# apache/datafusion-ballista

Hardware: NVIDIA H100
Metric: tpch_q1_rows_per_sec (higher is better)
Workload: dtype decimal128/i128

## Files before the change

datafusion-ballista_b200/csrc/host/engine.cpp:

```cpp
#include <sched.h>
#include <sys/stat.h>

#include <algorithm>
#include <atomic>
#include <cctype>
#include <chrono>
#include <cmath>
#include <cstdio>
#include <map>
#include <mutex>
#include <functional>
#include <set>

#include "../common/arrow_host.hpp"
#include "../common/tpch_gen.hpp"
#include "../device/kernels.h"
#include "host_pool.hpp"
#include "lower.hpp"
#include "nccl_dyn.hpp"
#include "../common/plan_proto.hpp"
#include "../common/plan_dump.hpp"
#include "parquet_meta.hpp"
#include "arrow_ipc.hpp"

// ... 25 lines not shown
  std::string name;
  uint64_t output_rows = 0, input_rows = 0, elapsed_ns = 0, bytes_read = 0, bytes_written = 0, launches = 0;
};

}

struct b200_engine {
  int device = 0;
  int rank = 0, world = 1;
  int sm_count = 132;
  cudaStream_t own_stream = nullptr;
  cudaStream_t stream = nullptr;
  std::mutex mu;
  std::map<std::string, std::map<int, DevBatchPtr>> tables;
  std::map<ShuffleKey, std::vector<Piece>> shuffle;
  std::atomic<uint64_t> launches{0};
  std::atomic<uint64_t> n_fused{0}, n_fused_static{0}, n_vm{0}, n_groupby{0}, n_groupby_pf{0}, n_fastfilter{0};
  int64_t batch_size = 8192;
  std::map<std::string, std::string> config;
  std::map<std::string, int> agg_hint;
  uint64_t pf_bucket_slots = (uint64_t)1 << 19;
  int64_t pf_min_rows = (int64_t)1 << 22;
  std::map<std::string, uint64_t> agg_groups;
  void* pinned_stage = nullptr;
  std::unique_ptr<HostPool> pool;
  std::mutex ingest_mu;
  struct NarrowSlot {
    void* pinned = nullptr;
    void* dev = nullptr;
    cudaEvent_t done = nullptr;
    bool used = false;
    size_t bytes = 0;
  } nslot[4];
  int64_t ingest_chunk_rows = (int64_t)1 << 22;
  int ingest_slots = 3;
  bool kernel_timing = false;
  struct KernelSample { std::string name; cudaEvent_t e0, e1; uint64_t bytes; };
  std::vector<KernelSample> ksamples;
  struct KernelStat { double ms = 0; uint64_t launches = 0, bytes = 0; };
  std::map<std::string, KernelStat> kstats;
  ncclComm_t comm = nullptr;
  std::mutex comm_mu;
  uint64_t exch_sent_bytes = 0, exch_recv_bytes = 0;
  size_t win_config_bytes = 0;
  uint8_t* win_local = nullptr;
  size_t win_bytes = 0, win_used = 0;
  std::vector<uint8_t*> win_peer;
  uint64_t fused_exchanges = 0;
  std::mutex export_mu;
  uint8_t* export_arena = nullptr;
  std::atomic<uint64_t> narrowed_bytes_saved{0};
  std::atomic<uint64_t> n_window_sorts{0};
  std::atomic<uint64_t> nlj_pairs{0};
};

struct b200_stage {
  b200_engine* eng = nullptr;
  std::string job_id;
  int64_t stage_id = 0;
  PlanPtr plan;
  std::string fingerprint;
  std::vector<OpMetrics> metrics;
  std::map<const PlanNode*, int> metric_index;
};

#define NCCL_CHECK(expr)                                                                                              \
  do {                                                                                                                \
    ncclResult_t _r = (expr);                                                                                         \
    if (_r != 0) throw EngineError(B200_ERR_CUDA, std::string("NCCL error: ") + NcclApi::get().GetErrorString(_r) + " at " + __FILE__ + ":" + std::to_string(__LINE__)); \
  } while (0)

static void release_window(b200_engine* e);
static void setup_window(b200_engine* e);

namespace {

struct TaskCtx {
  uint8_t* arena = nullptr;
  size_t pos = 0;
  bool drained = true;
  std::vector<std::function<void()>> checks;
};
static const size_t TASK_ARENA_BYTES = (size_t)1 << 16;
inline TaskCtx& task_ctx() {
  static thread_local TaskCtx t;
  if (!t.arena && cudaHostAlloc((void**)&t.arena, TASK_ARENA_BYTES, cudaHostAllocDefault) != cudaSuccess) t.arena = nullptr;
  return t;
}

struct Exec {
  b200_engine* e;
  b200_stage* s;
  const volatile int32_t* cancel;
  cudaStream_t st() const { return e->stream; }
  void check_cancel() const {
    if (cancel && *cancel) throw EngineError(B200_ERR_CANCELLED, "task cancelled");
  }
  OpMetrics* m(const PlanNode* n) const {
    if (!s) return nullptr;
    auto it = s->metric_index.find(n);
    return it == s->metric_index.end() ? nullptr : &s->metrics[(size_t)it->second];
  }
  const void* fetch_bytes(const void* dptr, size_t bytes) const {
    TaskCtx& t = task_ctx();
    if (!t.arena) throw EngineError(B200_ERR_OOM, "pinned read-back arena unavailable");
    if (t.drained) {
      t.pos = 0;
      t.drained = false;
    }
    const size_t at = (t.pos + 15) & ~(size_t)15;
    if (at + bytes > TASK_ARENA_BYTES) {
      sync();
      return fetch_bytes(dptr, bytes);
    }
    CUDA_CHECK(cudaMemcpyAsync(t.arena + at, dptr, bytes, cudaMemcpyDeviceToHost, st()));
    t.pos = at + bytes;
    return t.arena + at;
  }
  void* stage_bytes(size_t bytes) const {
    TaskCtx& t = task_ctx();
    if (!t.arena) throw EngineError(B200_ERR_OOM, "pinned staging arena unavailable");
    if (t.drained) {
      t.pos = 0;
      t.drained = false;
    }
    size_t at = (t.pos + 15) & ~(size_t)15;
    if (at + bytes > TASK_ARENA_BYTES) {
      sync();
      t.pos = 0;
      t.drained = false;
      at = 0;
      if (bytes > TASK_ARENA_BYTES) throw EngineError(B200_ERR_INVALID, "staging request larger than the arena");
    }
    t.pos = at + bytes;
    return t.arena + at;
  }
  template <class T>
  const T* fetch(const void* dptr) const {
    return (const T*)fetch_bytes(dptr, sizeof(T));
  }
  void defer(std::function<void()> fn) const { task_ctx().checks.push_back(std::move(fn)); }
  void sync() const {
    TaskCtx& t = task_ctx();
    cudaError_t se = cudaStreamSynchronize(st());
    t.drained = true;
    std::vector<std::function<void()>> cs;
    cs.swap(t.checks);
    CUDA_CHECK(se);
    for (auto& c : cs) c();
    check_cancel();
  }
  static void abandon() {
    TaskCtx& t = task_ctx();
    t.checks.clear();
    t.drained = true;
  }
  template <class T>
  T get(const void* dptr) const {
    const T* p = fetch<T>(dptr);
    sync();
    return *p;
  }
};

struct KernelTimer {
  b200_engine* e;
  cudaStream_t st;
  b200_engine::KernelSample ks;
  bool on;
  KernelTimer(const Exec& x, const char* name, uint64_t bytes) : e(x.e), st(x.st()), on(x.e->kernel_timing) {
    if (!on) return;
    ks.name = name;
    ks.bytes = bytes;
    if (cudaEventCreate(&ks.e0) != cudaSuccess || cudaEventCreate(&ks.e1) != cudaSuccess) {
      on = false;
      return;
    }
    cudaEventRecord(ks.e0, st);
  }
  ~KernelTimer() {
    if (!on) return;
    cudaEventRecord(ks.e1, st);
    std::lock_guard<std::mutex> g(e->mu);
    e->ksamples.push_back(ks);
  }
};

struct ScopeTimer {
  const char* name;
  std::chrono::steady_clock::time_point t0;
  bool on;
  explicit ScopeTimer(const char* n) : name(n) {
    static const bool enabled = getenv("B200_TIMING") != nullptr;
    on = enabled;
    if (on) t0 = std::chrono::steady_clock::now();
  }
  ~ScopeTimer() {
// ... 449 lines not shown
    if (hcs[ci].type.id == TypeId::Utf8) {
      int32_t total = 0;
      memcpy(&total, arena + slots[ci].data + (size_t)n * 4, 4);
      if ((size_t)total > slots[ci].chars_cap) return false;
    }
  for (size_t ci = 0; ci < b.cols.size(); ci++) {
    HostCol& h = hcs[ci];
    const Slot& sl = slots[ci];
    if (sl.has_valid) {
      unsigned long long nulls = 0;
      memcpy(&nulls, arena + sl.count, 8);
      h.null_count = (int64_t)nulls;
      if (nulls) h.validity.assign(arena + sl.validity, arena + sl.validity + (size_t)(n + 7) / 8);
    }
    if (!h.data.empty()) memcpy(h.data.data(), arena + sl.data, h.data.size());
    if (h.type.id == TypeId::Utf8) {
      const int32_t total = ((const int32_t*)h.data.data())[n];
      h.extra.assign(arena + sl.chars, arena + sl.chars + (size_t)total);
    }
  }
  hcs_out = std::move(hcs);
  return true;
}

std::vector<HostCol> download_batch(const Exec& x, const DevBatch& b, int64_t r0, int64_t r1) {
  const int64_t n = r1 - r0;
  std::vector<HostCol> hcs;
  if (n <= SMALL_EXPORT_ROWS && download_small(x, b, r0, r1, hcs)) return hcs;
  hcs.clear();
  cudaStream_t st = x.st();
  for (auto& c0 : b.cols) {
    DevColumn c = slice_column(c0, r0, r1);
    HostCol h;
    h.name = c.name;
    h.type = c.type;
    h.nullable = true;
    h.n = n;
    if (c.valid && n) {
      DevPtr bm = dev_alloc((size_t)(n + 7) / 8 + 16, st);
      DevPtr cnt = dev_alloc(8, st);
      CUDA_CHECK(cudaMemsetAsync(cnt->ptr, 0, 8, st));
      launch_bytes_to_bitmap(c.valid, (uint8_t*)bm->ptr, n, (unsigned long long*)cnt->ptr, st);
      h.validity.resize((size_t)(n + 7) / 8);
      CUDA_CHECK(cudaMemcpyAsync(h.validity.data(), bm->ptr, h.validity.size(), cudaMemcpyDeviceToHost, st));
      h.null_count = (int64_t)x.get<unsigned long long>(cnt->ptr);
      if (h.null_count == 0) h.validity.clear();
    }
    if (c.type.id == TypeId::Bool) {
      h.data.assign((size_t)(n + 7) / 8, 0);
      if (n) {
        DevPtr bm = dev_alloc((size_t)(n + 7) / 8 + 16, st);
        launch_bytes_to_bitmap(c.data, (uint8_t*)bm->ptr, n, nullptr, st);
        CUDA_CHECK(cudaMemcpyAsync(h.data.data(), bm->ptr, h.data.size(), cudaMemcpyDeviceToHost, st));
        CUDA_CHECK(cudaStreamSynchronize(st));
      }
    } else if (c.type.id == TypeId::Utf8) {
      DevColumn u = c.phys == PH_STRVIEW ? as_utf8(x, c) : c;
      h.data.resize((size_t)(n + 1) * 4);
      CUDA_CHECK(cudaMemcpyAsync(h.data.data(), u.data, h.data.size(), cudaMemcpyDeviceToHost, st));
      CUDA_CHECK(cudaStreamSynchronize(st));
      int32_t* off = (int32_t*)h.data.data();
      int32_t first = off[0], last = off[n];
      h.extra.resize((size_t)(last - first));
      if (last > first) CUDA_CHECK(cudaMemcpyAsync(h.extra.data(), u.chars + first, h.extra.size(), cudaMemcpyDeviceToHost, st));
      CUDA_CHECK(cudaStreamSynchronize(st));
      for (int64_t i = 0; i <= n; i++) off[i] -= first;
    } else {
      h.data.resize((size_t)n * c.width());
      if (n) CUDA_CHECK(cudaMemcpyAsync(h.data.data(), c.data, h.data.size(), cudaMemcpyDeviceToHost, st));
      CUDA_CHECK(cudaStreamSynchronize(st));
    }
    hcs.push_back(std::move(h));
  }
  return hcs;
}

void export_batch(const Exec& x, const DevBatch& b, int64_t r0, int64_t r1, ArrowArray* out, ArrowSchema* out_schema) {
  std::vector<HostCol> hcs = download_batch(x, b, r0, r1);
  export_record_batch(std::move(hcs), r1 - r0, out, out_schema);
}

struct RunOutcome {
  RunStatus status;
  float ms = 0;
};

struct FusedPlan {
  FusedSpec spec;
  FusedShape shape;
  int block = 0;
  size_t smem = 0;
};

static void throw_run_error(unsigned int error) {
  if (error == 1) throw EngineError(B200_ERR_EXECUTION, "Arithmetic overflow");
  if (error == 2) throw EngineError(B200_ERR_EXECUTION, "Divide by zero");
  if (error) throw EngineError(B200_ERR_EXECUTION, "execution error in expression");
}

static bool program_filters(const Program& P) {
  for (int i = 0; i < P.n_instr; i++)
    if (P.code[i].op == OP_FILTER || (P.code[i].flags & IF_FILTER)) return true;
  return false;
}

bool match_groupby(const Program& P, GroupBySpec& S);
bool match_fast_filter(const Program& P, FastFilterSpec& S);

bool partition_for_groupby(const Exec& x, GroupBySpec& S, std::vector<DevPtr>& keep) {
  const uint64_t GB_PF_BUCKET_SLOTS = x.e->pf_bucket_slots;
  if (!GB_PF_BUCKET_SLOTS || S.n_keys < 1 || S.table.cap < GB_PF_BUCKET_SLOTS * 8 || S.n_rows < x.e->pf_min_rows || S.n_rows >= ((int64_t)1 << 32)) return false;
  for (int k = 0; k < S.n_keys; k++) {
    const uint32_t w = S.cols[S.key_col[k]].width;
    if (w != 4 && w != 8) return false;
  }
  const uint32_t K = (uint32_t)std::min<uint64_t>(S.table.cap / GB_PF_BUCKET_SLOTS, PART_MAX_FANOUT);
  const int64_t n = S.n_rows;
  PidSrc ps;
  memset(&ps, 0, sizeof ps);
  ps.salt = 0x5bd1e995;
  for (int k = 0; k < S.n_keys; k++) {
    const FusedCol& c = S.cols[S.key_col[k]];
    ps.keys[ps.n_keys++] = KeyCol{c.data, nullptr, (uint8_t)(c.width == 4 ? PH_I32 : PH_I64), (uint8_t)c.width};
// ... 1616 lines not shown
      case PlanNode::Passthrough:
        out = (n.op_name == "CoalescePartitionsExec") ? exec_all(*n.children[0]) : exec(*n.children[0], part);
        break;
      case PlanNode::Limit: {
        DevBatchPtr in = (n.op_name == "GlobalLimitExec") ? exec_all(*n.children[0]) : exec(*n.children[0], part);
        int64_t r0 = std::min<int64_t>(std::max<int64_t>(0, n.skip), in->n);
        int64_t r1 = n.fetch >= 0 ? std::min<int64_t>(in->n, r0 + n.fetch) : in->n;
        out = std::make_shared<DevBatch>();
        out->n = r1 - r0;
        for (auto& c : in->cols) out->cols.push_back(slice_column(c, r0, r1));
        break;
      }
      case PlanNode::Window: out = exec_window(n, part, met); break;
      case PlanNode::ShuffleWriter: throw EngineError(B200_ERR_INVALID, "nested ShuffleWriterExec");
    }
    if (met) met->output_rows += (uint64_t)out->n;
    return out;
  }

  DevBatchPtr do_sort(const std::vector<SortKey>& keys, int64_t fetch, DevBatchPtr in, OpMetrics* met) {
    const int64_t n = in->n;
    auto t0 = std::chrono::steady_clock::now();
    std::vector<DevColumn> kcols;
    bool need_eval = false;
    for (auto& k : keys) need_eval |= k.expr->kind != Expr::Col;
    DevBatchPtr work = in;
    size_t n_in_cols = in->cols.size();
    if (need_eval && n > 0) {
      PipelineBuilder pb(*in, x.st());
      std::vector<ColRef> outs = pb.cols;
      for (auto& k : keys) {
        ColRef c = pb.compile(*k.expr);
        pb.pin(c);
        outs.push_back(c);
      }
      work = run_materialize(x, pb, outs, in, met);
      for (size_t k = 0; k < keys.size(); k++) kcols.push_back(work->cols[n_in_cols + k]);
    } else {
      for (auto& k : keys) kcols.push_back(in->cols.at((size_t)(k.expr->kind == Expr::Col ? k.expr->col : 0)));
    }
    if (n <= 1 || keys.empty()) {
      auto out = std::make_shared<DevBatch>();
      int64_t m = fetch >= 0 ? std::min<int64_t>(fetch, n) : n;
      out->n = m;
      for (size_t c = 0; c < n_in_cols; c++) out->cols.push_back(slice_column(in->cols[c], 0, m));
      return out;
    }
    const int64_t m = fetch >= 0 ? std::min<int64_t>(fetch, n) : n;
    DevPtr idx = sort_permutation(keys, kcols, n, m);
    DevBatch proj;
    proj.n = n;
    for (size_t c = 0; c < n_in_cols; c++) proj.cols.push_back(in->cols[c]);
    DevBatchPtr out = gather_batch(x, proj, (const int64_t*)idx->ptr, m, false);
    if (n > SMALL_SORT_MAX_ROWS || keys.size() > (size_t)SMALL_SORT_MAX_KEYS) CUDA_CHECK(cudaStreamSynchronize(x.st()));
    if (met) {
      met->elapsed_ns += (uint64_t)std::chrono::duration_cast<std::chrono::nanoseconds>(std::chrono::steady_clock::now() - t0).count();
      met->input_rows += (uint64_t)n;
    }
    return out;
  }

  static bool window_input_sorted(const PlanNode& n) {
    const PlanNode* c = n.children[0].get();
    while (c->op == PlanNode::Passthrough && c->op_name == "CoalesceBatchesExec") c = c->children[0].get();
    if (c->op != PlanNode::Sort && c->op != PlanNode::SortPreservingMerge) return false;
    const size_t np = n.window_partition.size(), no = n.window_order.size();
    if (c->sort_keys.size() != np + no) return false;
    auto in_sort_prefix = [&](const ExprPtr& e) {
      for (size_t k = 0; k < np; k++)
        if (expr_equal(c->sort_keys[k].expr, e)) return true;
      return false;
    };
    for (size_t k = 0; k < np; k++) {
      bool found = false;
      for (auto& pk : n.window_partition) found = found || expr_equal(c->sort_keys[k].expr, pk);
      if (!found || !in_sort_prefix(n.window_partition[k])) return false;
    }
    for (size_t k = 0; k < no; k++) {
      const SortKey &a = c->sort_keys[np + k], &b = n.window_order[k];
      if (!expr_equal(a.expr, b.expr) || a.asc != b.asc || a.nulls_first != b.nulls_first) return false;
    }
    return true;
  }

  DevBatchPtr exec_window(const PlanNode& n, int part, OpMetrics* met) {
    DevBatchPtr in = exec(*n.children[0], part);
    const auto t0 = std::chrono::steady_clock::now();
    const int64_t N = in->n;
    if (N >= ((int64_t)1 << 32)) throw EngineError(B200_ERR_UNSUPPORTED, "window over " + std::to_string(N) + " rows (the sort takes at most 2^32)");
    const size_t np = n.window_partition.size(), no = n.window_order.size(), nw = n.window_exprs.size();
    if (np + no > (size_t)WIN_MAX_KEYS) throw EngineError(B200_ERR_UNSUPPORTED, "window with more than " + std::to_string(WIN_MAX_KEYS) + " partition and order keys");
    auto out = std::make_shared<DevBatch>();
    out->n = N;
    out->cols = in->cols;
    const size_t n_in = in->cols.size();
    if (met) met->input_rows += (uint64_t)N;
    if (N == 0) {
      for (size_t w = 0; w < nw; w++) {
        const Field& f = n.schema[n_in + w];
        DevColumn c = make_out_column(f.name, f.type, f.type.id == TypeId::Utf8 ? PH_STRVIEW : phys_of(f.type), 0, f.nullable, x.st());
        c.n = 0;
        out->cols.push_back(c);
      }
      return out;
    }
    std::vector<ExprPtr> exprs(n.window_partition);
    for (auto& k : n.window_order) exprs.push_back(k.expr);
// ... 213 lines not shown
      }
      DevPtr fv, fc, bv, bc, tiles;
      {
        KernelTimer kt(x, "window_scan", (uint64_t)N * ((arg ? (uint64_t)arg->width() + 1 : 0) + (perm ? 8 : 0) + vw + 1) +
                                             (uint64_t)N * (fwd + bwd) * 2 * (vw + 1 + 8 + vw + 4));
        launch_window_load(L, perm, N, x.st());
        WinScan S;
        memset(&S, 0, sizeof S);
        S.vals = vals->ptr;
        S.valid = (const uint8_t*)valid->ptr;
        S.n = N;
        S.w = std::max<int64_t>(E.w, 1);
        S.acc = E.acc;
        S.op = E.op;
        S.seg = seg;
        if (fwd || bwd) tiles = dev_alloc((size_t)window_scan_tile_bytes(N), x.st());
        S.tiles = tiles ? tiles->ptr : nullptr;
        if (fwd) {
          fv = dev_alloc((size_t)N * vw, x.st());
          fc = dev_alloc((size_t)N * 4, x.st());
          S.out_v = fv->ptr;
          S.out_c = (uint32_t*)fc->ptr;
          S.dir = 0;
          launch_window_scan(S, B, x.st());
          E.fwd_v = fv->ptr;
          E.fwd_c = (const uint32_t*)fc->ptr;
        }
        x.check_cancel();
        if (bwd) {
          bv = dev_alloc((size_t)N * vw, x.st());
          bc = dev_alloc((size_t)N * 4, x.st());
          S.out_v = bv->ptr;
          S.out_c = (uint32_t*)bc->ptr;
          S.dir = 1;
          launch_window_scan(S, B, x.st());
          E.bwd_v = bv->ptr;
          E.bwd_c = (const uint32_t*)bc->ptr;
        }
      }
      if (E.fin == WFIN_AVG && E.acc == WACC_I128) {
        if (!error) {
          error = dev_alloc(16, x.st());
          CUDA_CHECK(cudaMemsetAsync(error->ptr, 0, 16, x.st()));
        }
        E.error = (unsigned int*)error->ptr;
      }
      {
        KernelTimer kt(x, "window_frames", (uint64_t)N * (32 + 2 * (vw + 4) + (perm ? 8 : 0) + (uint64_t)oc.width() + 1));
        launch_window_eval(E, B, perm, N, x.st());
      }
      out->cols.push_back(oc);
    }
    if (error && x.get<unsigned int>(error->ptr)) throw EngineError(B200_ERR_EXECUTION, "Arithmetic overflow in a window AVG over Decimal128");
    CUDA_CHECK(cudaStreamSynchronize(x.st()));
    if (met) met->elapsed_ns += (uint64_t)std::chrono::duration_cast<std::chrono::nanoseconds>(std::chrono::steady_clock::now() - t0).count();
    return out;
  }

  DevPtr sort_permutation(const std::vector<SortKey>& keys, const std::vector<DevColumn>& kcols, int64_t n, int64_t m) {
    if (n >= ((int64_t)1 << 32)) throw EngineError(B200_ERR_UNSUPPORTED, "sort of more than 2^32 rows");
    if (n <= SMALL_SORT_MAX_ROWS && keys.size() <= (size_t)SMALL_SORT_MAX_KEYS) {
      SmallSortKeys K;
      K.n_keys = (int)keys.size();
      std::vector<DevColumn> kv;
      for (size_t ki = 0; ki < keys.size(); ki++) {
        kv.push_back(as_views(x, kcols[ki]));
        const DevColumn& kc = kv.back();
        SortWordArgs& A = K.k[ki];
        A.data = kc.data;
        A.valid = kc.valid;
        A.phys = kc.phys;
        A.asc = keys[ki].asc;
        A.nulls_first = keys[ki].nulls_first;
        A.word = 0;
      }
      DevPtr idx = dev_alloc((size_t)n * 8, x.st());
      launch_small_sort(K, (int64_t*)idx->ptr, n, x.st());
      return idx;
    }
    const uint32_t n_blocks = (uint32_t)((n + 2047) / 2048);
    DevPtr ka = dev_alloc((size_t)n * 8, x.st()), kb = dev_alloc((size_t)n * 8, x.st());
    DevPtr va = dev_alloc((size_t)n * 4, x.st()), vb = dev_alloc((size_t)n * 4, x.st());
    DevPtr hist = dev_alloc((size_t)256 * n_blocks * 4 + 64, x.st());
    DevPtr scan = dev_alloc(((size_t)256 * n_blocks + 1 + (size_t)(256 * n_blocks) / 1024 + 8) * 8, x.st());
    uint32_t* perm = (uint32_t*)va->ptr;
    launch_iota_u32(perm, n, x.st());
    for (size_t ki = keys.size(); ki-- > 0;) {
      DevColumn kc = as_views(x, kcols[ki]);
      int n_words = 1;
      if (kc.phys == PH_DEC128) n_words = 2;
      if (kc.phys == PH_STRVIEW) {
        DevPtr mx = dev_alloc(16, x.st());
        CUDA_CHECK(cudaMemsetAsync(mx->ptr, 0, 16, x.st()));
        launch_max_view_len((const unsigned long long*)kc.data, kc.valid, n, (unsigned int*)mx->ptr, x.st());
        unsigned int maxlen = x.get<unsigned int>(mx->ptr);
        n_words = (int)(maxlen / 7) + 1;
      }
      for (int w = n_words - 1; w >= (kc.valid ? -1 : 0); w--) {
        x.check_cancel();
        SortWordArgs A;
        A.data = kc.data;
        A.valid = kc.valid;
        A.phys = kc.phys;
        A.asc = keys[ki].asc;
        A.nulls_first = keys[ki].nulls_first;
        A.word = w;
        uint64_t* kin = (uint64_t*)ka->ptr;
// ... 1687 lines not shown
    return B200_OK;
  } catch (const EngineError& e) {
    g_err = e.what();
    return e.code;
  } catch (const PlanUnsupported& e) {
    g_err = e.what();
    return B200_ERR_UNSUPPORTED;
  } catch (const std::bad_alloc&) {
    g_err = "host out of memory";
    return B200_ERR_OOM;
  } catch (const std::exception& e) {
    g_err = e.what();
    return B200_ERR_INVALID;
  } catch (...) {
    g_err = "unknown error";
    return B200_ERR_INVALID;
  }
}

template <class F>
int guard(b200_engine* e, F&& f) {
  const uint64_t l0 = launches_on_thread();
  const int rc = guard(std::forward<F>(f));
  if (e) e->launches += launches_on_thread() - l0;
  return rc;
}

}

static void release_window(b200_engine* e) {
  for (size_t d = 0; d < e->win_peer.size(); d++)
    if (e->win_peer[d] && (int)d != e->rank) cudaIpcCloseMemHandle(e->win_peer[d]);
  e->win_peer.clear();
  if (e->win_local) cudaFree(e->win_local);
  e->win_local = nullptr;
  e->win_bytes = e->win_used = 0;
}

static void comm_allgather(b200_engine* e, const void* mine, void* all, size_t rec) {
  NcclApi& N = NcclApi::get();
  const int W = e->world, me = e->rank;
  uint8_t* dev = nullptr;
  CUDA_CHECK(cudaMalloc((void**)&dev, rec * (size_t)W));
  try {
    CUDA_CHECK(cudaMemcpyAsync(dev + rec * (size_t)me, mine, rec, cudaMemcpyHostToDevice, e->stream));
    NCCL_CHECK(N.GroupStart());
    for (int d = 0; d < W; d++) {
      if (d == me) continue;
      NCCL_CHECK(N.Send(dev + rec * (size_t)me, rec, kNcclUint8, d, e->comm, e->stream));
      NCCL_CHECK(N.Recv(dev + rec * (size_t)d, rec, kNcclUint8, d, e->comm, e->stream));
    }
    NCCL_CHECK(N.GroupEnd());
    CUDA_CHECK(cudaMemcpyAsync(all, dev, rec * (size_t)W, cudaMemcpyDeviceToHost, e->stream));
    CUDA_CHECK(cudaStreamSynchronize(e->stream));
  } catch (...) {
    cudaFree(dev);
    throw;
  }
  cudaFree(dev);
}

static void setup_window(b200_engine* e) {
  const int W = e->world, me = e->rank;
  struct Rec {
    cudaIpcMemHandle_t h;
    uint64_t bytes, ok;
  };
  Rec mine;
  memset(&mine, 0, sizeof mine);
  const size_t want = (e->win_config_bytes + 4095) & ~(size_t)4095;
  uint8_t* ptr = nullptr;
  if (cudaMalloc((void**)&ptr, want) == cudaSuccess && cudaIpcGetMemHandle(&mine.h, ptr) == cudaSuccess) {
    mine.bytes = want;
    mine.ok = 1;
  } else {
    cudaGetLastError();
    if (ptr) cudaFree(ptr);
    ptr = nullptr;
  }
  std::vector<Rec> all((size_t)W);
  comm_allgather(e, &mine, all.data(), sizeof(Rec));
  bool ok = true;
  for (auto& r : all) ok = ok && r.ok && r.bytes == want;
  std::vector<uint8_t*> peer((size_t)W, nullptr);
  if (ok) {
    for (int d = 0; d < W && ok; d++) {
      if (d == me) {
        peer[(size_t)d] = ptr;
        continue;
      }
      void* m = nullptr;
      if (cudaIpcOpenMemHandle(&m, all[(size_t)d].h, cudaIpcMemLazyEnablePeerAccess) != cudaSuccess) {
        cudaGetLastError();
        ok = false;
      }
      peer[(size_t)d] = (uint8_t*)m;
    }
  }
  uint64_t flag = ok ? 1 : 0;
  std::vector<uint64_t> flags((size_t)W, 0);
  comm_allgather(e, &flag, flags.data(), sizeof flag);
  for (uint64_t f : flags) ok = ok && f;
  if (!ok) {
    for (int d = 0; d < W; d++)
      if (d != me && peer[(size_t)d]) cudaIpcCloseMemHandle(peer[(size_t)d]);
    if (ptr) cudaFree(ptr);
    return;
// ... 72 lines not shown
    CUDA_CHECK(cudaDeviceGetDefaultMemPool(&pool, device));
    uint64_t thr = pool_bytes ? pool_bytes : UINT64_MAX;
    CUDA_CHECK(cudaMemPoolSetAttribute(pool, cudaMemPoolAttrReleaseThreshold, &thr));
    *out = e;
  });
}

void b200_engine_destroy(b200_engine* e) {
  if (!e) return;
  cudaSetDevice(e->device);
  cudaStreamSynchronize(e->stream);
  e->tables.clear();
  e->shuffle.clear();
  cudaStreamSynchronize(e->stream);
  for (auto& sl : e->nslot) {
    if (sl.pinned) cudaFreeHost(sl.pinned);
    if (sl.dev) cudaFree(sl.dev);
    if (sl.done) cudaEventDestroy(sl.done);
  }
  release_window(e);
  if (e->comm && NcclApi::get().ok()) NcclApi::get().CommDestroy(e->comm);
  if (e->export_arena) cudaFreeHost(e->export_arena);
  if (arena_chunk() && arena_chunk()->stream == e->own_stream) arena_chunk().reset();
  if (e->own_stream) cudaStreamDestroy(e->own_stream);
  delete e;
}

int b200_engine_set_stream(b200_engine* e, void* cuda_stream) {
  return guard([&] {
    CUDA_CHECK(cudaStreamSynchronize(e->stream));
    e->stream = cuda_stream ? (cudaStream_t)cuda_stream : e->own_stream;
  });
}
int b200_engine_synchronize(b200_engine* e) {
  return guard([&] {
    CUDA_CHECK(cudaSetDevice(e->device));
    CUDA_CHECK(cudaStreamSynchronize(e->stream));
  });
}
uint64_t b200_engine_kernel_launches(b200_engine* e) { return e->launches; }
uint64_t b200_engine_counter(b200_engine* e, const char* name) {
  const std::string n = name ? name : "";
  if (n == "fused") return e->n_fused;
  if (n == "groupby_partition_first") return e->n_groupby_pf;
  if (n == "fused_static") return e->n_fused_static;
  if (n == "fused_exchanges") return e->fused_exchanges;
  if (n == "exchange_window_bytes") return e->win_bytes;
  if (n == "vm") return e->n_vm;
  if (n == "groupby") return e->n_groupby;
  if (n == "fastfilter") return e->n_fastfilter;
  if (n == "ingest_bytes_saved") return e->narrowed_bytes_saved;
  if (n == "nlj_pairs") return e->nlj_pairs;
  if (n == "window_sorts") return e->n_window_sorts;
  return 0;
}

int b200_engine_set_config(b200_engine* e, const char* key, const char* value) {
  return guard([&] {
    std::lock_guard<std::mutex> g(e->mu);
    e->config[key] = value;
    if (std::string(key) == "datafusion.execution.batch_size") e->batch_size = std::max<int64_t>(1, atoll(value));
    if (std::string(key) == "b200.ingest.chunk_rows") e->ingest_chunk_rows = std::max<int64_t>(1 << 16, atoll(value));
    if (std::string(key) == "b200.ingest.slots") e->ingest_slots = atoi(value);
    if (std::string(key) == "b200.exchange.window_bytes") e->win_config_bytes = (size_t)strtoull(value, nullptr, 10);
    if (std::string(key) == "b200.ingest.threads") e->pool.reset();
    if (std::string(key) == "b200.agg.partition_first.bucket_slots") {
      const uint64_t v = strtoull(value, nullptr, 10);
      e->pf_bucket_slots = v ? std::max<uint64_t>(next_pow2(v), 64) : 0;
    }
    if (std::string(key) == "b200.agg.partition_first.min_rows") e->pf_min_rows = std::max<int64_t>(1, atoll(value));
    if (std::string(key) == "b200.agg.reset_hints") {
      e->agg_hint.clear();
      e->agg_groups.clear();
    }
    if (std::string(key) == "b200.metrics.kernel_timing") e->kernel_timing = std::string(value) == "on" || std::string(value) == "1" || std::string(value) == "true";
  });
}

int b200_engine_register_batch(b200_engine* e, const char* table, int partition, struct ArrowArray* batch, struct ArrowSchema* schema) {
  return guard(e, [&] {
    CUDA_CHECK(cudaSetDevice(e->device));
    DevBatchPtr b = import_batch(e, batch, schema);
    Exec x{e, nullptr, nullptr};
    build_column_images(x, *b);
    DevBatchPtr prev;
    {
      std::lock_guard<std::mutex> g(e->mu);
      auto& slot = e->tables[table][partition];
      prev = slot;
      if (!prev) slot = b;
    }
    if (prev) {
      Runner r{x, ""};
      Schema s;
      for (auto& c : prev->cols) s.push_back(Field{c.name, c.type, true});
      DevBatchPtr cat = r.concat({prev, b}, s);
      for (auto& c : cat->cols) c = as_utf8(x, c);
      build_column_images(x, *cat);
      CUDA_CHECK(cudaStreamSynchronize(e->stream));
      std::lock_guard<std::mutex> g(e->mu);
      e->tables[table][partition] = cat;
    }
  });
}

int b200_engine_drop_table(b200_engine* e, const char* table) {
// ... 154 lines not shown
int b200_engine_register_parquet(b200_engine* e, const char* table, int partition, const char* path, const char* columns_csv) {
  return guard(e, [&] {
    if (!e || !table || !path) throw EngineError(B200_ERR_INVALID, "null argument");
    CUDA_CHECK(cudaSetDevice(e->device));
    std::vector<std::string> cols;
    if (columns_csv && *columns_csv) {
      std::string sct(columns_csv);
      size_t p = 0;
      while (p <= sct.size()) {
        size_t q = sct.find(',', p);
        if (q == std::string::npos) q = sct.size();
        if (q > p) cols.push_back(sct.substr(p, q - p));
        p = q + 1;
      }
    }
    Exec x{e, nullptr, nullptr};
    DevBatchPtr b;
    try {
      b = scan_parquet(x, path, cols);
    } catch (...) {
      cudaStreamSynchronize(e->stream);
      Exec::abandon();
      throw;
    }
    std::lock_guard<std::mutex> g(e->mu);
    e->tables[table][partition] = b;
  });
}

int64_t b200_tpch_table_rows(const char* table, int64_t msf) {
  const int t = table ? table_id(table) : -1;
  return t < 0 ? -1 : tpch::table_rows(t, msf);
}

int b200_engine_export_table(b200_engine* e, const char* table, int partition, struct ArrowArray* out, struct ArrowSchema* out_schema) {
  return guard(e, [&] {
    CUDA_CHECK(cudaSetDevice(e->device));
    DevBatchPtr b;
    {
      std::lock_guard<std::mutex> g(e->mu);
      auto it = e->tables.find(table);
      if (it == e->tables.end() || !it->second.count(partition)) throw EngineError(B200_ERR_NOT_FOUND, "no such table partition");
      b = it->second[partition];
    }
    Exec x{e, nullptr, nullptr};
    export_batch(x, *b, 0, b->n, out, out_schema);
  });
}

int b200_stage_prepare(b200_engine* e, const char* job_id, int64_t stage_id, const char* plan_json, uint64_t plan_len, b200_stage** out) {
  ScopeTimer tm("stage_prepare");
  return guard([&] {
    if (!e || !plan_json || !out) throw EngineError(B200_ERR_INVALID, "null argument");
    Json j = parse_json(plan_json, plan_len ? (size_t)plan_len : strlen(plan_json));
    PlanPtr plan = parse_plan(j);
    if (plan->op != PlanNode::ShuffleWriter)
      throw EngineError(B200_ERR_INVALID, "Plan passed to new_query_stage_exec is not a ShuffleWriterExec");
    auto* s = new b200_stage();
    s->eng = e;
    s->job_id = job_id ? job_id : plan->job_id;
    s->stage_id = stage_id;
    plan->stage_id = stage_id;
    {
      std::string shape(plan_json, plan_len ? (size_t)plan_len : strlen(plan_json));
      const std::string tag = "\"job_id\":\"";
      size_t at = shape.find(tag);
      if (at != std::string::npos) {
        size_t end = shape.find('"', at + tag.size());
        if (end != std::string::npos) shape.erase(at + tag.size(), end - at - tag.size());
      }
      s->fingerprint = std::to_string(stage_id) + ":" + std::to_string(mix64(hash_bytes((const uint8_t*)shape.data(), (uint32_t)shape.size())));
    }
    collect_nodes(*plan, s);
    s->plan = std::move(plan);
    *out = s;
  });
}

int b200_plan_proto_to_json(const void* plan_bytes, uint64_t n_bytes, const char* job_id, char** out_json) {
  return guard([&] {
    if (!plan_bytes || !out_json) throw EngineError(B200_ERR_INVALID, "null argument");
    std::string js;
    try {
      js = pbp::plan_proto_to_json(plan_bytes, (size_t)n_bytes, job_id ? std::string(job_id) : std::string());
    } catch (const pbp::Unsupported& u) {
      throw EngineError(B200_ERR_UNSUPPORTED, u.what());
    } catch (const std::runtime_error& r) {
      throw EngineError(B200_ERR_INVALID, r.what());
    }
    char* m = (char*)malloc(js.size() + 1);
    if (!m) throw EngineError(B200_ERR_OOM, "plan JSON");
    memcpy(m, js.c_str(), js.size() + 1);
    *out_json = m;
  });
}

void b200_string_free(char* s) { free(s); }

int b200_plan_typed_json(const char* plan_json, uint64_t plan_len, char** out_json) {
  return guard([&] {
    if (!plan_json || !out_json) throw EngineError(B200_ERR_INVALID, "null argument");
    Json j = parse_json(plan_json, plan_len ? (size_t)plan_len : strlen(plan_json));
    PlanPtr plan = parse_plan(j);
    const std::string js = dump_plan(*plan);
    char* m = (char*)malloc(js.size() + 1);
    if (!m) throw EngineError(B200_ERR_OOM, "plan JSON");
    memcpy(m, js.c_str(), js.size() + 1);
    *out_json = m;
  });
}

int b200_stage_prepare_proto(b200_engine* e, const char* job_id, int64_t stage_id, const void* plan_bytes, uint64_t n_bytes, b200_stage** out) {
  char* js = nullptr;
  int rc = b200_plan_proto_to_json(plan_bytes, n_bytes, job_id, &js);
  if (rc != 0) return rc;
  rc = b200_stage_prepare(e, job_id, stage_id, js, 0, out);
  free(js);
  return rc;
}

int b200_stage_prepare_task(b200_engine* e, const void* task_bytes, uint64_t n_bytes, int multi, b200_stage** out_stage, char** out_task_json) {
  std::string job;
  int64_t stage_id = 0;
  pbp::Slice plan;
  int rc = guard([&] {
// ... 63 lines not shown
        f.msg(5, fe);
      } else if (r->status == B200_ERR_CANCELLED) {
        f.str(1, msg.empty() ? std::string("Task killed") : msg);
        f.msg(9, pbp::Writer());
      } else {
        f.str(1, "Task failed due to runtime execution error: " + msg);
        f.msg(4, pbp::Writer());
      }
      w.msg(10, f);
    }
    for (int i = 0; i < n_metrics; i++) {
      pbp::Writer set;
      auto one = [&](uint32_t field, uint64_t v) {
        pbp::Writer m;
        m.u64_always(field, v);
        set.msg(1, m);
      };
      auto named = [&](const char* name, uint64_t v) {
        pbp::Writer nc;
        nc.str(1, name);
        nc.u64(2, v);
        pbp::Writer m;
        m.msg(6, nc);
        set.msg(1, m);
      };
      one(1, metrics[i].output_rows);
      one(2, metrics[i].elapsed_compute_ns);
      one(12, metrics[i].bytes_written);
      named("input_rows", metrics[i].input_rows);
      named("bytes_read", metrics[i].bytes_read);
      named("kernel_launches", metrics[i].kernel_launches);
      w.msg(12, set);
    }
    char* m = (char*)malloc(w.out.size() + 1);
    if (!m) throw EngineError(B200_ERR_OOM, "task status");
    memcpy(m, w.out.data(), w.out.size());
    m[w.out.size()] = 0;
    *out_bytes = m;
    *out_len = w.out.size();
  });
}

int b200_stage_execute(b200_stage* s, int input_partition, const volatile int32_t* cancel_flag, b200_shuffle_write_partition* out, int cap, int* n_out) {
  ScopeTimer tm("stage_execute");
  return guard(s ? s->eng : nullptr, [&] {
    if (!s || !n_out) throw EngineError(B200_ERR_INVALID, "null argument");
    CUDA_CHECK(cudaSetDevice(s->eng->device));
    Exec x{s->eng, s, cancel_flag};
    Runner r{x, s->job_id};
    std::vector<b200_shuffle_write_partition> res;
    try {
      res = r.execute_stage(*s->plan, input_partition);
    } catch (...) {
      cudaStreamSynchronize(s->eng->stream);
      Exec::abandon();
      {
        std::lock_guard<std::mutex> g(s->eng->mu);
        for (auto it = s->eng->shuffle.begin(); it != s->eng->shuffle.end();) {
          if (it->first.job == s->job_id && it->first.stage == s->stage_id) {
            auto& v = it->second;
            v.erase(std::remove_if(v.begin(), v.end(), [&](const Piece& pc) { return (pc.file_id == input_partition || (pc.file_id < 0 && it->first.part == input_partition)) && pc.src_rank == s->eng->rank; }), v.end());
            if (v.empty()) {
              it = s->eng->shuffle.erase(it);
              continue;
            }
          }
          ++it;
        }
      }
      throw;
    }
    if ((int)res.size() > cap) throw EngineError(B200_ERR_INVALID, "output array too small");
    for (size_t i = 0; i < res.size(); i++) out[i] = res[i];
    *n_out = (int)res.size();
  });
}

int b200_stage_execute_exchange(b200_stage* s, int input_partition, const volatile int32_t* cancel_flag, b200_shuffle_write_partition* out, int cap,
                                int* n_out, b200_exchange_stats* stats) {
  ScopeTimer tm("stage_execute_exchange");
  return guard(s ? s->eng : nullptr, [&] {
    if (!s || !n_out) throw EngineError(B200_ERR_INVALID, "null argument");
    b200_engine* e = s->eng;
    if (s->plan->op != PlanNode::ShuffleWriter || s->plan->n_out_partitions < 1)
      throw EngineError(B200_ERR_INVALID, "b200_stage_execute_exchange needs a hash-partitioning ShuffleWriterExec");
    CUDA_CHECK(cudaSetDevice(e->device));
    Exec x{e, s, cancel_flag};
    Runner r{x, s->job_id};
    Runner::FusedExchange fx;
    std::vector<b200_shuffle_write_partition> res;
    uint64_t sent = 0, recvd = 0;
    try {
      res = r.execute_stage(*s->plan, input_partition, &fx);
      if (fx.done) {
        sent = fx.sent;
        recvd = fx.recvd;
      } else if (e->world > 1) {
        Exchange ex{x, Runner{x, s->job_id}, e, s->job_id, s->stage_id, (int)s->plan->n_out_partitions, EXCH_HASH, 0, s->plan->schema, s->plan->schema.size()};
        ex.run(&sent, &recvd);
      }
    } catch (...) {
      cudaStreamSynchronize(e->stream);
      Exec::abandon();
      throw;
    }
    e->exch_sent_bytes += sent;
    e->exch_recv_bytes += recvd;
    if (stats) {
      stats->sent_bytes = sent;
      stats->recv_bytes = recvd;
    }
    if ((int)res.size() > cap) throw EngineError(B200_ERR_INVALID, "output array too small");
    for (size_t i = 0; i < res.size(); i++) out[i] = res[i];
    *n_out = (int)res.size();
  });
}

int b200_stage_metrics(b200_stage* s, b200_operator_metrics* out, int cap, int* n_out) {
  return guard([&] {
    int n = (int)std::min<size_t>(s->metrics.size(), (size_t)cap);
    for (int i = 0; i < n; i++) {
      memset(&out[i], 0, sizeof out[i]);
      snprintf(out[i].name, sizeof out[i].name, "%s", s->metrics[(size_t)i].name.c_str());
      out[i].output_rows = s->metrics[(size_t)i].output_rows;
      out[i].input_rows = s->metrics[(size_t)i].input_rows;
      out[i].elapsed_compute_ns = s->metrics[(size_t)i].elapsed_ns;
      out[i].bytes_read = s->metrics[(size_t)i].bytes_read;
      out[i].bytes_written = s->metrics[(size_t)i].bytes_written;
      out[i].kernel_launches = s->metrics[(size_t)i].launches;
    }
    *n_out = n;
  });
}

void b200_stage_release(b200_stage* s) { delete s; }

int b200_partition_export(b200_engine* e, const char* job_id, int64_t stage_id, int out_partition, struct ArrowArray* out, struct ArrowSchema* out_schema) {
  ScopeTimer tm("partition_export");
  return guard(e, [&] {
    CUDA_CHECK(cudaSetDevice(e->device));
    std::vector<std::pair<DevBatchPtr, std::pair<int64_t, int64_t>>> pieces;
    {
      std::lock_guard<std::mutex> g(e->mu);
      auto it = e->shuffle.find(ShuffleKey{job_id, stage_id, out_partition});
      if (it == e->shuffle.end()) throw EngineError(B200_ERR_NOT_FOUND, "no such shuffle partition");
      for (auto& p : it->second) pieces.push_back({p.batch, {p.r0, p.r1}});
    }
    Exec x{e, nullptr, nullptr};
    if (pieces.size() == 1) {
      export_batch(x, *pieces[0].first, pieces[0].second.first, pieces[0].second.second, out, out_schema);
      return;
    }
    Runner r{x, job_id};
    Schema s;
    for (auto& c : pieces[0].first->cols) s.push_back(Field{c.name, c.type, true});
// ... 63 lines not shown
      k++;
    }
    *n_out = k;
    if (reset) e->kstats.clear();
  });
}


int b200_comm_unique_id(void* out, uint64_t cap) {
  return guard([&] {
    if (!out || cap < sizeof(ncclUniqueId)) throw EngineError(B200_ERR_INVALID, "b200_comm_unique_id needs a 128-byte buffer");
    NcclApi& N = NcclApi::get();
    if (!N.ok()) throw EngineError(B200_ERR_CUDA, "libnccl not available: " + N.error);
    ncclUniqueId id;
    NCCL_CHECK(N.GetUniqueId(&id));
    memcpy(out, &id, sizeof id);
  });
}

int b200_engine_comm_init(b200_engine* e, const void* nccl_id, uint64_t id_bytes) {
  return guard([&] {
    if (!e || !nccl_id || id_bytes < sizeof(ncclUniqueId)) throw EngineError(B200_ERR_INVALID, "b200_engine_comm_init: bad arguments");
    if (e->world <= 1) return;
    NcclApi& N = NcclApi::get();
    if (!N.ok()) throw EngineError(B200_ERR_CUDA, "libnccl not available: " + N.error);
    CUDA_CHECK(cudaSetDevice(e->device));
    std::lock_guard<std::mutex> g(e->comm_mu);
    if (e->comm) {
      N.CommDestroy(e->comm);
      e->comm = nullptr;
    }
    ncclUniqueId id;
    memcpy(&id, nccl_id, sizeof id);
    NCCL_CHECK(N.CommInitRank(&e->comm, e->world, id, e->rank));
    release_window(e);
    if (e->win_config_bytes) setup_window(e);
  });
}

int b200_exchange_stage(b200_engine* e, const char* job_id, int64_t stage_id, int n_out_partitions, int mode, int root, const char* schema_json,
                        b200_exchange_stats* stats) {
  return guard(e, [&] {
    if (!e || !job_id || !schema_json) throw EngineError(B200_ERR_INVALID, "null argument");
    if (mode < 0 || mode > 2 || n_out_partitions < 0 || root < 0 || root >= std::max(e->world, 1)) throw EngineError(B200_ERR_INVALID, "b200_exchange_stage: bad mode / root");
    CUDA_CHECK(cudaSetDevice(e->device));
    Json j = parse_json(schema_json, strlen(schema_json));
    Exec x{e, nullptr, nullptr};
    Exchange ex{x, Runner{x, job_id}, e, job_id, stage_id, n_out_partitions, mode, root, parse_schema(j), 0};
    ex.ncols = ex.schema.size();
    uint64_t sent = 0, recvd = 0;
    try {
      ex.run(&sent, &recvd);
    } catch (...) {
      cudaStreamSynchronize(e->stream);
      Exec::abandon();
      throw;
    }
    e->exch_sent_bytes += sent;
    e->exch_recv_bytes += recvd;
    if (stats) {
      stats->sent_bytes = sent;
      stats->recv_bytes = recvd;
    }
  });
}

static std::vector<HostCol> host_cols_from_arrow(ArrowArray* arr, ArrowSchema* sch, int64_t* n_rows) {
  std::vector<ImportedCol> ics = import_record_batch(arr, sch, n_rows);
  const int64_t n = *n_rows;
  std::vector<HostCol> out;
  for (auto& ic : ics) {
    HostCol h;
    h.name = ic.name;
    h.type = ic.type;
    h.nullable = ic.nullable;
    h.n = n;
    if (ic.large_offsets) throw EngineError(B200_ERR_UNSUPPORTED, "LargeUtf8 columns are not supported");
    auto bit = [](const uint8_t* bm, int64_t i) { return (bm[i >> 3] >> (i & 7)) & 1; };
    if (ic.null_count > 0 && ic.validity) {
      h.validity.assign((size_t)((n + 7) / 8), 0);
      for (int64_t i = 0; i < n; i++)
        if (bit(ic.validity, i + ic.offset)) h.validity[(size_t)(i >> 3)] |= (uint8_t)(1u << (i & 7));
        else h.null_count++;
      if (h.null_count == 0) h.validity.clear();
    }
    if (ic.type.id == TypeId::Null) {
      h.null_count = n;
    } else if (ic.type.id == TypeId::Bool) {
      h.data.assign((size_t)((n + 7) / 8), 0);
      for (int64_t i = 0; i < n; i++)
        if (bit(ic.data, i + ic.offset)) h.data[(size_t)(i >> 3)] |= (uint8_t)(1u << (i & 7));
    } else if (ic.type.id == TypeId::Utf8) {
      const int32_t* off = (const int32_t*)ic.data + ic.offset;
      h.data.resize((size_t)(n + 1) * 4);
      int32_t* po = (int32_t*)h.data.data();
      for (int64_t i = 0; i <= n; i++) po[i] = off[i] - off[0];
      if (n) h.extra.assign(ic.extra + off[0], ic.extra + off[n]);
    } else {
      const size_t w = (size_t)ic.type.width();
      h.data.assign(ic.data + (size_t)ic.offset * w, ic.data + (size_t)(ic.offset + n) * w);
    }
    out.push_back(std::move(h));
  }
  return out;
}

static std::vector<uint8_t> read_whole_file(const std::string& path, uint64_t offset, uint64_t length) {
// ... 208 lines not shown
```

datafusion-ballista_b200/engine.py:

```python
from __future__ import annotations

import ctypes as C
import os
from typing import List, Optional

import pyarrow as pa

_PKG = os.path.dirname(os.path.abspath(__file__))
LIB_PATH = os.environ.get("B200EXEC_LIB") or os.path.join(_PKG, "lib", "libb200exec.so")


class ShuffleWritePartition(C.Structure):
    _fields_ = [("partition_id", C.c_uint64), ("num_batches", C.c_uint64), ("num_rows", C.c_uint64),
                ("num_bytes", C.c_uint64), ("file_id", C.c_int64), ("is_sort_shuffle", C.c_int32),
                ("_pad", C.c_int32)]

    def as_tuple(self):
        return (self.partition_id, self.num_batches, self.num_rows, self.num_bytes, self.file_id, self.is_sort_shuffle)


class OperatorMetrics(C.Structure):
    _fields_ = [("name", C.c_char * 48), ("output_rows", C.c_uint64), ("input_rows", C.c_uint64),
                ("elapsed_compute_ns", C.c_uint64), ("bytes_read", C.c_uint64), ("bytes_written", C.c_uint64),
                ("kernel_launches", C.c_uint64)]


class KernelStat(C.Structure):
    _fields_ = [("name", C.c_char * 48), ("elapsed_ns", C.c_uint64), ("launches", C.c_uint64), ("algorithmic_bytes", C.c_uint64)]


class ExchangeStats(C.Structure):
    _fields_ = [("sent_bytes", C.c_uint64), ("recv_bytes", C.c_uint64)]


EXCHANGE_HASH, EXCHANGE_GATHER, EXCHANGE_BROADCAST = 0, 1, 2
NCCL_ID_BYTES = 128


class ArrowSchema(C.Structure):
    _fields_ = [("format", C.c_char_p), ("name", C.c_char_p), ("metadata", C.c_char_p), ("flags", C.c_int64),
                ("n_children", C.c_int64), ("children", C.c_void_p), ("dictionary", C.c_void_p),
                ("release", C.c_void_p), ("private_data", C.c_void_p)]


class ArrowArray(C.Structure):
    _fields_ = [("length", C.c_int64), ("null_count", C.c_int64), ("offset", C.c_int64), ("n_buffers", C.c_int64),
                ("n_children", C.c_int64), ("buffers", C.c_void_p), ("children", C.c_void_p),
                ("dictionary", C.c_void_p), ("release", C.c_void_p), ("private_data", C.c_void_p)]


EXPORTED_SYMBOLS = [
    "b200_engine_create", "b200_engine_destroy", "b200_last_error", "b200_engine_set_stream",
    "b200_engine_synchronize", "b200_engine_kernel_launches", "b200_engine_counter", "b200_engine_set_config",
    "b200_engine_register_batch", "b200_engine_register_parquet", "b200_parquet_describe", "b200_engine_drop_table", "b200_engine_tpch_generate",
    "b200_engine_export_table", "b200_tpch_table_rows", "b200_stage_prepare", "b200_stage_execute", "b200_stage_metrics",
    "b200_stage_release", "b200_partition_export", "b200_partition_rows",
# ... 63 lines not shown
    L.b200_comm_unique_id.argtypes = [vp, u64]
    L.b200_engine_comm_init.argtypes = [vp, vp, u64]
    L.b200_exchange_stage.argtypes = [vp, cp, i64, ci, ci, ci, cp, C.POINTER(ExchangeStats)]
    L.b200_stage_execute_exchange.argtypes = [vp, ci, vp, C.POINTER(ShuffleWritePartition), ci, C.POINTER(ci), C.POINTER(ExchangeStats)]
    L.b200_host_alloc_pinned.argtypes = [u64]
    L.b200_host_alloc_pinned.restype = vp
    L.b200_host_free_pinned.argtypes = [vp]
    L.b200_host_free_pinned.restype = None
    L.b200_version.restype = cp
    _lib = L
    return L


class B200Error(RuntimeError):
    NAMES = {-1: "Plan", -2: "NotImplemented", -3: "Execution", -4: "External(CUDA)", -5: "FetchFailed",
             -6: "Cancelled", -7: "ResourcesExhausted"}

    def __init__(self, code, msg):
        super().__init__(f"{self.NAMES.get(code, code)}: {msg}")
        self.code = code


def _check(rc):
    if rc != 0:
        raise B200Error(rc, load_library().b200_last_error().decode(errors="replace"))


def ipc_encode(batch: pa.RecordBatch, compress: bool = True, max_rows_per_message: int = 0) -> bytes:
    arr, sch = ArrowArray(), ArrowSchema()
    batch._export_to_c(C.addressof(arr), C.addressof(sch))
    out, n = C.c_void_p(), C.c_uint64(0)
    _check(load_library().b200_ipc_encode(C.addressof(arr), C.addressof(sch), 1 if compress else 0, max_rows_per_message, C.byref(out), C.byref(n)))
    try:
        return C.string_at(out.value, n.value)
    finally:
        load_library().b200_ipc_free(out)


def ipc_decode(data: bytes) -> pa.RecordBatch:
    arr, sch = ArrowArray(), ArrowSchema()
    buf = C.create_string_buffer(data, len(data))
    _check(load_library().b200_ipc_decode(buf, len(data), C.addressof(arr), C.addressof(sch)))
    return pa.RecordBatch._import_from_c(C.addressof(arr), C.addressof(sch))


def parquet_describe(path: str) -> dict:
    import json as _json
    cap = 1 << 20
    buf = C.create_string_buffer(cap)
    _check(load_library().b200_parquet_describe(path.encode(), buf, cap))
    return _json.loads(buf.value.decode())


class QueryStageExecutor:
    def __init__(self, engine: "GpuExecutionEngine", handle, job_id: str, stage_id: int):
        self.engine, self.h, self.job_id, self.stage_id = engine, handle, job_id, stage_id
        self._cap = 8192
        self._out = (ShuffleWritePartition * self._cap)()

    def execute_query_stage(self, input_partition: int, cancel_flag=None) -> List[ShuffleWritePartition]:
        cap = self._cap
        out = self._out
        n = C.c_int(0)
        cf = C.addressof(cancel_flag) if cancel_flag is not None else None
        _check(load_library().b200_stage_execute(self.h, input_partition, cf, out, cap, C.byref(n)))
        res = [ShuffleWritePartition.from_buffer_copy(out[i]) for i in range(n.value)]
        return res

    def execute_query_stage_exchange(self, input_partition: int, cancel_flag=None):
        n = C.c_int(0)
        st = ExchangeStats()
        cf = C.addressof(cancel_flag) if cancel_flag is not None else None
        _check(load_library().b200_stage_execute_exchange(self.h, input_partition, cf, self._out, self._cap, C.byref(n), C.byref(st)))
        res = [ShuffleWritePartition.from_buffer_copy(self._out[i]) for i in range(n.value)]
        return res, {"sent_bytes": st.sent_bytes, "recv_bytes": st.recv_bytes}

    def collect_plan_metrics(self) -> List[dict]:
        cap = 256
        out = (OperatorMetrics * cap)()
        n = C.c_int(0)
        _check(load_library().b200_stage_metrics(self.h, out, cap, C.byref(n)))
        return [dict(name=out[i].name.decode(), output_rows=out[i].output_rows, input_rows=out[i].input_rows,
                     elapsed_compute_ns=out[i].elapsed_compute_ns, bytes_read=out[i].bytes_read,
                     bytes_written=out[i].bytes_written, kernel_launches=out[i].kernel_launches)
                for i in range(n.value)]

    def release(self):
        if self.h:
            load_library().b200_stage_release(self.h)
            self.h = None


def plan_proto_to_json(plan_bytes: bytes, job_id: Optional[str] = None) -> str:
    L = load_library()
    out = C.c_void_p()
    buf = C.create_string_buffer(plan_bytes, len(plan_bytes))
    _check(L.b200_plan_proto_to_json(C.cast(buf, C.c_void_p), len(plan_bytes), job_id.encode() if job_id else None, C.byref(out)))
    try:
        return C.string_at(out.value).decode()
    finally:
        L.b200_string_free(out)


class TaskResult(C.Structure):
    _fields_ = [("task_id", C.c_uint32), ("stage_id", C.c_uint32), ("stage_attempt_num", C.c_uint32), ("partition_id", C.c_uint32),
                ("launch_time", C.c_uint64), ("start_exec_time", C.c_uint64), ("end_exec_time", C.c_uint64), ("status", C.c_int32),
                ("fetch_map_stage_id", C.c_uint32), ("fetch_map_partition_id", C.c_uint32), ("fetch_executor_id", C.c_char_p),
                ("error_message", C.c_char_p)]


def task_status_encode(job_id: str, executor_id: str, result: "TaskResult", partitions=(), metrics=()) -> bytes:
    L = load_library()
    parts = (ShuffleWritePartition * max(len(partitions), 1))(*partitions)
    mets = (OperatorMetrics * max(len(metrics), 1))(*metrics)
    out, n = C.c_void_p(), C.c_uint64(0)
    _check(L.b200_task_status_encode(job_id.encode(), executor_id.encode(), C.byref(result), parts, len(partitions), mets, len(metrics),
                                     C.byref(out), C.byref(n)))
    try:
        return C.string_at(out.value, n.value)
    finally:
        L.b200_string_free(out)


def task_definition_decode(task_bytes: bytes, multi: bool = False) -> dict:
    import json as _json
    L = load_library()
    out = C.c_void_p()
    buf = C.create_string_buffer(task_bytes, len(task_bytes))
    _check(L.b200_stage_prepare_task(None, C.cast(buf, C.c_void_p), len(task_bytes), 1 if multi else 0, None, C.byref(out)))
    try:
        return _json.loads(C.string_at(out.value).decode())
    finally:
        L.b200_string_free(out)

# ... 172 lines not shown
```

Before: 35.06 billion.

## Cache parsed stage plans by shape and reuse per-thread ctypes output buffers

```diff
diff --git a/datafusion-ballista_b200/csrc/host/engine.cpp b/datafusion-ballista_b200/csrc/host/engine.cpp
--- a/datafusion-ballista_b200/csrc/host/engine.cpp
+++ b/datafusion-ballista_b200/csrc/host/engine.cpp
@@ -101,13 +101,15 @@
   std::atomic<uint64_t> narrowed_bytes_saved{0};
   std::atomic<uint64_t> n_window_sorts{0};
   std::atomic<uint64_t> nlj_pairs{0};
+  std::atomic<uint64_t> host_syncs{0};
+  std::map<std::string, std::shared_ptr<const PlanNode>> plan_cache;
 };
 
 struct b200_stage {
   b200_engine* eng = nullptr;
   std::string job_id;
   int64_t stage_id = 0;
-  PlanPtr plan;
+  std::shared_ptr<const PlanNode> plan;
   std::string fingerprint;
   std::vector<OpMetrics> metrics;
   std::map<const PlanNode*, int> metric_index;
@@ -137,6 +139,11 @@
   return t;
 }
 
+inline cudaError_t host_wait(b200_engine* e, cudaStream_t st) {
+  e->host_syncs++;
+  return cudaStreamSynchronize(st);
+}
+
 struct Exec {
   b200_engine* e;
   b200_stage* s;
@@ -191,7 +198,7 @@
   void defer(std::function<void()> fn) const { task_ctx().checks.push_back(std::move(fn)); }
   void sync() const {
     TaskCtx& t = task_ctx();
-    cudaError_t se = cudaStreamSynchronize(st());
+    cudaError_t se = host_wait(e, st());
     t.drained = true;
     std::vector<std::function<void()>> cs;
     cs.swap(t.checks);
@@ -747,23 +754,23 @@
         DevPtr bm = dev_alloc((size_t)(n + 7) / 8 + 16, st);
         launch_bytes_to_bitmap(c.data, (uint8_t*)bm->ptr, n, nullptr, st);
         CUDA_CHECK(cudaMemcpyAsync(h.data.data(), bm->ptr, h.data.size(), cudaMemcpyDeviceToHost, st));
-        CUDA_CHECK(cudaStreamSynchronize(st));
+        CUDA_CHECK(host_wait(x.e, st));
       }
     } else if (c.type.id == TypeId::Utf8) {
       DevColumn u = c.phys == PH_STRVIEW ? as_utf8(x, c) : c;
       h.data.resize((size_t)(n + 1) * 4);
       CUDA_CHECK(cudaMemcpyAsync(h.data.data(), u.data, h.data.size(), cudaMemcpyDeviceToHost, st));
-      CUDA_CHECK(cudaStreamSynchronize(st));
+      CUDA_CHECK(host_wait(x.e, st));
       int32_t* off = (int32_t*)h.data.data();
       int32_t first = off[0], last = off[n];
       h.extra.resize((size_t)(last - first));
       if (last > first) CUDA_CHECK(cudaMemcpyAsync(h.extra.data(), u.chars + first, h.extra.size(), cudaMemcpyDeviceToHost, st));
-      CUDA_CHECK(cudaStreamSynchronize(st));
+      CUDA_CHECK(host_wait(x.e, st));
       for (int64_t i = 0; i <= n; i++) off[i] -= first;
     } else {
       h.data.resize((size_t)n * c.width());
       if (n) CUDA_CHECK(cudaMemcpyAsync(h.data.data(), c.data, h.data.size(), cudaMemcpyDeviceToHost, st));
-      CUDA_CHECK(cudaStreamSynchronize(st));
+      CUDA_CHECK(host_wait(x.e, st));
     }
     hcs.push_back(std::move(h));
   }
@@ -2486,7 +2493,7 @@
     proj.n = n;
     for (size_t c = 0; c < n_in_cols; c++) proj.cols.push_back(in->cols[c]);
     DevBatchPtr out = gather_batch(x, proj, (const int64_t*)idx->ptr, m, false);
-    if (n > SMALL_SORT_MAX_ROWS || keys.size() > (size_t)SMALL_SORT_MAX_KEYS) CUDA_CHECK(cudaStreamSynchronize(x.st()));
+    if (n > SMALL_SORT_MAX_ROWS || keys.size() > (size_t)SMALL_SORT_MAX_KEYS) CUDA_CHECK(host_wait(x.e, x.st()));
     if (met) {
       met->elapsed_ns += (uint64_t)std::chrono::duration_cast<std::chrono::nanoseconds>(std::chrono::steady_clock::now() - t0).count();
       met->input_rows += (uint64_t)n;
@@ -2806,7 +2813,7 @@
       out->cols.push_back(oc);
     }
     if (error && x.get<unsigned int>(error->ptr)) throw EngineError(B200_ERR_EXECUTION, "Arithmetic overflow in a window AVG over Decimal128");
-    CUDA_CHECK(cudaStreamSynchronize(x.st()));
+    CUDA_CHECK(host_wait(x.e, x.st()));
     if (met) met->elapsed_ns += (uint64_t)std::chrono::duration_cast<std::chrono::nanoseconds>(std::chrono::steady_clock::now() - t0).count();
     return out;
   }
@@ -4600,7 +4607,7 @@
     }
     NCCL_CHECK(N.GroupEnd());
     CUDA_CHECK(cudaMemcpyAsync(all, dev, rec * (size_t)W, cudaMemcpyDeviceToHost, e->stream));
-    CUDA_CHECK(cudaStreamSynchronize(e->stream));
+    CUDA_CHECK(host_wait(e, e->stream));
   } catch (...) {
     cudaFree(dev);
     throw;
@@ -4779,6 +4786,7 @@
   if (n == "ingest_bytes_saved") return e->narrowed_bytes_saved;
   if (n == "nlj_pairs") return e->nlj_pairs;
   if (n == "window_sorts") return e->n_window_sorts;
+  if (n == "host_syncs") return e->host_syncs;
   return 0;
 }
 
@@ -5039,25 +5047,40 @@
   ScopeTimer tm("stage_prepare");
   return guard([&] {
     if (!e || !plan_json || !out) throw EngineError(B200_ERR_INVALID, "null argument");
-    Json j = parse_json(plan_json, plan_len ? (size_t)plan_len : strlen(plan_json));
-    PlanPtr plan = parse_plan(j);
-    if (plan->op != PlanNode::ShuffleWriter)
-      throw EngineError(B200_ERR_INVALID, "Plan passed to new_query_stage_exec is not a ShuffleWriterExec");
+    const size_t len = plan_len ? (size_t)plan_len : strlen(plan_json);
+    std::string shape(plan_json, len);
+    const std::string tag = "\"job_id\":\"";
+    size_t at = shape.find(tag);
+    if (at != std::string::npos) {
+      size_t end = shape.find('"', at + tag.size());
+      if (end != std::string::npos) shape.erase(at + tag.size(), end - at - tag.size());
+    }
+    const std::string cache_key = std::to_string(stage_id) + ":" + shape;
+    std::shared_ptr<const PlanNode> plan;
+    if (job_id) {
+      std::lock_guard<std::mutex> g(e->mu);
+      auto it = e->plan_cache.find(cache_key);
+      if (it != e->plan_cache.end()) plan = it->second;
+    }
+    if (!plan) {
+      Json j = parse_json(plan_json, len);
+      PlanPtr parsed = parse_plan(j);
+      if (parsed->op != PlanNode::ShuffleWriter)
+        throw EngineError(B200_ERR_INVALID, "Plan passed to new_query_stage_exec is not a ShuffleWriterExec");
+      parsed->stage_id = stage_id;
+      plan = std::shared_ptr<const PlanNode>(std::move(parsed));
+      if (job_id) {
+        static const size_t PLAN_CACHE_MAX = 256;
+        std::lock_guard<std::mutex> g(e->mu);
+        if (e->plan_cache.size() >= PLAN_CACHE_MAX) e->plan_cache.clear();
+        e->plan_cache.emplace(cache_key, plan);
+      }
+    }
     auto* s = new b200_stage();
     s->eng = e;
     s->job_id = job_id ? job_id : plan->job_id;
     s->stage_id = stage_id;
-    plan->stage_id = stage_id;
-    {
-      std::string shape(plan_json, plan_len ? (size_t)plan_len : strlen(plan_json));
-      const std::string tag = "\"job_id\":\"";
-      size_t at = shape.find(tag);
-      if (at != std::string::npos) {
-        size_t end = shape.find('"', at + tag.size());
-        if (end != std::string::npos) shape.erase(at + tag.size(), end - at - tag.size());
-      }
-      s->fingerprint = std::to_string(stage_id) + ":" + std::to_string(mix64(hash_bytes((const uint8_t*)shape.data(), (uint32_t)shape.size())));
-    }
+    s->fingerprint = std::to_string(stage_id) + ":" + std::to_string(mix64(hash_bytes((const uint8_t*)shape.data(), (uint32_t)shape.size())));
     collect_nodes(*plan, s);
     s->plan = std::move(plan);
     *out = s;
@@ -5227,7 +5250,7 @@
     try {
       res = r.execute_stage(*s->plan, input_partition);
     } catch (...) {
-      cudaStreamSynchronize(s->eng->stream);
+      host_wait(s->eng, s->eng->stream);
       Exec::abandon();
       {
         std::lock_guard<std::mutex> g(s->eng->mu);
@@ -5275,7 +5298,7 @@
         ex.run(&sent, &recvd);
       }
     } catch (...) {
-      cudaStreamSynchronize(e->stream);
+      host_wait(e, e->stream);
       Exec::abandon();
       throw;
     }
@@ -5445,7 +5468,7 @@
     try {
       ex.run(&sent, &recvd);
     } catch (...) {
-      cudaStreamSynchronize(e->stream);
+      host_wait(e, e->stream);
       Exec::abandon();
       throw;
     }
diff --git a/datafusion-ballista_b200/engine.py b/datafusion-ballista_b200/engine.py
--- a/datafusion-ballista_b200/engine.py
+++ b/datafusion-ballista_b200/engine.py
@@ -2,6 +2,7 @@
 
 import ctypes as C
 import os
+import threading
 from typing import List, Optional
 
 import pyarrow as pa
@@ -171,34 +172,50 @@
     return _json.loads(buf.value.decode())
 
 
+_out_bufs = threading.local()
+_OUT_CAP = 8192
+_METRICS_CAP = 256
+
+
+def _partition_buffer():
+    b = getattr(_out_bufs, "partitions", None)
+    if b is None:
+        b = _out_bufs.partitions = (ShuffleWritePartition * _OUT_CAP)()
+    return b
+
+
+def _metrics_buffer():
+    b = getattr(_out_bufs, "metrics", None)
+    if b is None:
+        b = _out_bufs.metrics = (OperatorMetrics * _METRICS_CAP)()
+    return b
+
+
 class QueryStageExecutor:
     def __init__(self, engine: "GpuExecutionEngine", handle, job_id: str, stage_id: int):
         self.engine, self.h, self.job_id, self.stage_id = engine, handle, job_id, stage_id
-        self._cap = 8192
-        self._out = (ShuffleWritePartition * self._cap)()
 
     def execute_query_stage(self, input_partition: int, cancel_flag=None) -> List[ShuffleWritePartition]:
-        cap = self._cap
-        out = self._out
+        out = _partition_buffer()
         n = C.c_int(0)
         cf = C.addressof(cancel_flag) if cancel_flag is not None else None
-        _check(load_library().b200_stage_execute(self.h, input_partition, cf, out, cap, C.byref(n)))
+        _check(load_library().b200_stage_execute(self.h, input_partition, cf, out, _OUT_CAP, C.byref(n)))
         res = [ShuffleWritePartition.from_buffer_copy(out[i]) for i in range(n.value)]
         return res
 
     def execute_query_stage_exchange(self, input_partition: int, cancel_flag=None):
         n = C.c_int(0)
         st = ExchangeStats()
+        out = _partition_buffer()
         cf = C.addressof(cancel_flag) if cancel_flag is not None else None
-        _check(load_library().b200_stage_execute_exchange(self.h, input_partition, cf, self._out, self._cap, C.byref(n), C.byref(st)))
-        res = [ShuffleWritePartition.from_buffer_copy(self._out[i]) for i in range(n.value)]
+        _check(load_library().b200_stage_execute_exchange(self.h, input_partition, cf, out, _OUT_CAP, C.byref(n), C.byref(st)))
+        res = [ShuffleWritePartition.from_buffer_copy(out[i]) for i in range(n.value)]
         return res, {"sent_bytes": st.sent_bytes, "recv_bytes": st.recv_bytes}
 
     def collect_plan_metrics(self) -> List[dict]:
-        cap = 256
-        out = (OperatorMetrics * cap)()
+        out = _metrics_buffer()
         n = C.c_int(0)
-        _check(load_library().b200_stage_metrics(self.h, out, cap, C.byref(n)))
+        _check(load_library().b200_stage_metrics(self.h, out, _METRICS_CAP, C.byref(n)))
         return [dict(name=out[i].name.decode(), output_rows=out[i].output_rows, input_rows=out[i].input_rows,
                      elapsed_compute_ns=out[i].elapsed_compute_ns, bytes_read=out[i].bytes_read,
                      bytes_written=out[i].bytes_written, kernel_launches=out[i].kernel_launches)
```

After: 41.79 billion (median of 6 runs). 1.19x the previous value.
